# vsergeev/luaradio

Hardware: AMD Instinct MI355X
Metric: MSamples/s per block (128-tap complex FIR headline) + WBFM chain end-to-end (higher is better)
Workload: dtype f32

## Files before the change

### luaradio_amd/csrc/kernels_channelizer.h

```cpp
#pragma once
#include "common.h"
#include "kernels_fir.h"

#ifndef LRHIP_CHAN_EXP
#define LRHIP_CHAN_EXP 0
#endif

namespace lrhip {

#ifndef LRHIP_CHAN_INTERLEAVE
#define LRHIP_CHAN_INTERLEAVE 1
#endif
#ifndef LRHIP_CHAN_RT
#define LRHIP_CHAN_RT 1
#endif
#ifndef LRHIP_CHAN_KSLAB
#define LRHIP_CHAN_KSLAB 32
#endif
constexpr int CHAN_RT = LRHIP_CHAN_RT;
constexpr int CHAN_MT = 64 * CHAN_RT;
constexpr int CHAN_KSLAB = LRHIP_CHAN_KSLAB;

template <int NCT>
__global__ __launch_bounds__(256, CHAN_RT == 1 ? 2 : 1) void channelizer_kernel(const float *__restrict__ hist, const float *__restrict__ x,
                                                             const float *__restrict__ W, float *__restrict__ y,
                                                             int M, long n, long nframes, long first)
{
    constexpr int K2 = 16 * NCT;
    constexpr int K = K2 / 2;
    constexpr int DROW = K2 + 2;
    constexpr int WROW = K2 + 16;
    extern __shared__ __attribute__((aligned(16))) float lds[];
    const int tid = threadIdx.x, lane = tid & 63, wave = tid >> 6;
    const int col = lane & 15, kq = lane >> 4;
    const long f0 = (long)blockIdx.x * CHAN_MT;
    const int nsamp = (CHAN_MT - 1) * K + M;
    const int nflt = 2 * nsamp;
    float *ldsD = lds;
    const int dsize = ((nflt + 2 * (nflt / K2) + 2 + 3) / 4) * 4;
    float *ldsW = lds + dsize;

    const long p0 = first + f0 * K;
    const long xlo = p0 - (M - 1);
    if (xlo >= 0 && xlo + nsamp <= n && ((reinterpret_cast<uintptr_t>(x + 2 * xlo) & 15) == 0)) {
        const float4 *src = reinterpret_cast<const float4 *>(x + 2 * xlo);
        for (int i4 = tid; i4 < nflt / 4; i4 += 256) {
            float4 v = src[i4];
            int a = 4 * i4, p = a + 2 * (a / K2);
            *reinterpret_cast<float2 *>(ldsD + p) = make_float2(v.x, v.y);
            *reinterpret_cast<float2 *>(ldsD + p + 2) = make_float2(v.z, v.w);
        }
        for (int a = (nflt / 4) * 4 + tid; a < nflt; a += 256) ldsD[a + 2 * (a / K2)] = x[2 * xlo + a];
    } else {
        for (int r = tid; r < nsamp; r += 256) {
            int a = 2 * r, p = a + 2 * (a / K2);
            ldsD[p] = stream_at<2>(hist, x, p0 + r, 0, M, n);
            ldsD[p + 1] = stream_at<2>(hist, x, p0 + r, 1, M, n);
        }
    }

    constexpr int SLAB_F4 = CHAN_KSLAB * K2 / 4;
    constexpr int UW = (SLAB_F4 + 255) / 256;
    const float4 *W4 = reinterpret_cast<const float4 *>(W);
    static_assert(UW <= 8, "W slab prefetch: at most 8 float4 per thread");
    float4 w0, w1, w2, w3, w4, w5, w6, w7;
#define LR_CHAN_FOR8(OP) OP(0) OP(1) OP(2) OP(3) OP(4) OP(5) OP(6) OP(7)
#define LR_CHAN_LOAD(U)                                                                          \
    if (U < UW) {                                                                                \
        int i4 = tid + U * 256;                                                                  \
        w##U = W4[wbase + (i4 < SLAB_F4 ? i4 : SLAB_F4 - 1)];                                    \
    }
#define LR_CHAN_PUT(U)                                                                           \
    if (U < UW) {                                                                                \
        int i4 = tid + U * 256;                                                                  \
        if (i4 < SLAB_F4) *reinterpret_cast<float4 *>(wdst + ((4 * i4) / K2) * WROW + (4 * i4) % K2) = w##U; \
    }
    {
        const size_t wbase = 0;
        float *wdst = ldsW;
        LR_CHAN_FOR8(LR_CHAN_LOAD)
        LR_CHAN_FOR8(LR_CHAN_PUT)
    }
    __syncthreads();

    f32x4 acc[CHAN_RT][NCT];
#pragma unroll
    for (int r = 0; r < CHAN_RT; r++)
#pragma unroll
        for (int c = 0; c < NCT; c++) acc[r][c] = (f32x4){0.f, 0.f, 0.f, 0.f};
    const float *abase = ldsD + DROW * (wave * 16 * CHAN_RT + col) + kq;
    const int nslabs = 2 * M / CHAN_KSLAB;
    for (int s = 0; s < nslabs; s++) {
        const float *wcur = ldsW + (s & 1) * (CHAN_KSLAB * WROW);
#if LRHIP_CHAN_EXP == 1
        const bool more = false;
#else
        const bool more = s + 1 < nslabs;
#endif
        if (more) {
            const size_t wbase = (size_t)(s + 1) * SLAB_F4;
            LR_CHAN_FOR8(LR_CHAN_LOAD)
        }
        const float *ap = abase + CHAN_KSLAB * s + 2 * ((CHAN_KSLAB * s) / K2);
        const float *bp = wcur + kq * WROW + col;
        constexpr int NST = CHAN_KSLAB / 4;
        float av[2][CHAN_RT], bv[2][NCT];
        auto fetch = [&](int buf, int st) {
#pragma unroll
            for (int r = 0; r < CHAN_RT; r++) av[buf][r] = ap[16 * r * DROW + 4 * st];
#pragma unroll
            for (int c = 0; c < NCT; c++) bv[buf][c] = bp[4 * st * WROW + 16 * c];
        };
        fetch(0, 0);
#pragma unroll
        for (int st = 0; st < NST; st++) {
#if LRHIP_CHAN_INTERLEAVE
            if (st + 1 < NST) fetch((st + 1) & 1, st + 1);
#pragma unroll
            for (int c = 0; c < NCT; c++)
#pragma unroll
                for (int r = 0; r < CHAN_RT; r++)
                    acc[r][c] = __builtin_amdgcn_mfma_f32_16x16x4f32(av[st & 1][r], bv[st & 1][c], acc[r][c], 0, 0, 0);
#pragma unroll
            for (int i = 0; i < NCT * CHAN_RT; i++) {
                __builtin_amdgcn_sched_group_barrier(0x008, 1, 0);
                __builtin_amdgcn_sched_group_barrier(0x100, 1, 0);
            }
            __builtin_amdgcn_sched_barrier(0);
#else
            if (st + 1 < NST) fetch((st + 1) & 1, st + 1);
            __builtin_amdgcn_sched_barrier(0);
#pragma unroll
            for (int c = 0; c < NCT; c++)
#pragma unroll
                for (int r = 0; r < CHAN_RT; r++)
                    acc[r][c] = __builtin_amdgcn_mfma_f32_16x16x4f32(av[st & 1][r], bv[st & 1][c], acc[r][c], 0, 0, 0);
            __builtin_amdgcn_sched_barrier(0);
#endif
        }
        if (more) {
            float *wdst = ldsW + ((s + 1) & 1) * (CHAN_KSLAB * WROW);
            LR_CHAN_FOR8(LR_CHAN_PUT)
        }
#if LRHIP_CHAN_EXP != 1
        __syncthreads();
#endif
    }

#pragma unroll
    for (int rt = 0; rt < CHAN_RT; rt++)
#pragma unroll
        for (int c = 0; c < NCT; c++)
#pragma unroll
            for (int r = 0; r < 4; r++) {
                long f = f0 + (wave * CHAN_RT + rt) * 16 + 4 * kq + r;
                if (f < nframes) y[f * K2 + 16 * c + col] = acc[rt][c][r];
            }
}

#undef LR_CHAN_FOR8
#undef LR_CHAN_LOAD
#undef LR_CHAN_PUT

}
```

### luaradio_amd/csrc/stage_pfb.h

```cpp
#pragma once

struct PfbChannelizerStage : lrhip_stage {
    int seek(unsigned long long, unsigned long long *) override { return set_error("seek: not supported by the channelizer stage"); }
    long memory() const override { return -1; }
    int M = 0, K = 0, log2k = 0, P = 0, R = 1, D = 0;
    DeviceBuf taps, tw, hist[2];
    int cur = 0;
    unsigned long index = 0;
    unsigned phase = 0;
    const char *kind() const override { return "pfb_channelizer"; }
    unsigned long max_output(unsigned long n) const override { return (n / D + 1) * K; }
    static const char *refusal(unsigned ntaps, unsigned nchannels)
    {
        if (nchannels < 8 || nchannels > 4096 || (nchannels & (nchannels - 1))) return "pfb_channelizer: nchannels must be a power of two in [8, 4096]";
        const unsigned hi = 64 * nchannels < 65536 ? 64 * nchannels : 65536;
        if (ntaps < nchannels || ntaps > hi) return "pfb_channelizer: ntaps must be in [nchannels, min(64 * nchannels, 65536)]";
        return nullptr;
    }
    static const char *refusal(unsigned ntaps, unsigned nchannels, unsigned oversample)
    {
        if (oversample != 1 && oversample != 2 && oversample != 4) return "pfb_channelizer: oversample must be 1, 2 or 4";
        return refusal(ntaps, nchannels);
    }
    int frames_per_tile() const { return K <= 256 ? PFB_TILE_SMALL / K : K == 512 ? 8 : K == 1024 ? 4 : PFB_TILE_LARGE / K; }
    int frames_per_group() const { return K <= 1024 ? frames_per_tile() : PFB_SCRATCH / K; }
    int reset() override
    {
        cur = 0; index = 0; phase = 0;
        size_t hb = (size_t)(M - 1) * 2 * sizeof(float);
        return (zero_fill(hist[0], hb) || zero_fill(hist[1], hb)) ? -1 : 0;
    }
    template <int F, int NT>
    int launch(const float *x, long n, float *y, long nframes)
    {
        const int T = frames_per_tile(), G = frames_per_group();
        size_t lds_bytes = ((size_t)(T + G) * K + K / 2) * sizeof(float2);
        auto kern = pfb_channelizer_kernel<F, NT>;
        if (kernel_allow_lds(kern, lds_bytes)) return -1;
        unsigned grid = (unsigned)((nframes + T - 1) / T);
        hipLaunchKernelGGL(kern, dim3(grid), dim3(NT), lds_bytes, ctx().stream, (const float *)hist[cur].p, x, (const float *)taps.p,
                           (const float2 *)tw.p, y, M, log2k, P, T, G, n, nframes, (long)index);
        LR_LAUNCH_CHECK();
        return 0;
    }
    template <int RR, int F, int NT>
    int launch_oversampled(int T, int G, const float *x, long n, float *y, long nframes)
    {
        if (F > 1 && T % (RR * F)) return set_error("pfb_channelizer: a tile of %d frames does not hold blocks of %d frames in %d classes", T, F, RR);
        size_t lds_bytes = ((size_t)(T + G) * K + K / 2) * sizeof(float2);
        auto kern = pfb_oversampled_kernel<RR, F, NT>;
        if (kernel_allow_lds(kern, lds_bytes)) return -1;
        unsigned grid = (unsigned)((nframes + T - 1) / T);
        hipLaunchKernelGGL(kern, dim3(grid), dim3(NT), lds_bytes, ctx().stream, (const float *)hist[cur].p, x, (const float *)taps.p,
                           (const float2 *)tw.p, y, M, log2k, P, T, G, n, nframes, (long)index, (int)phase);
        LR_LAUNCH_CHECK();
        return 0;
    }
    int launch_oversampled_by_k(const float *x, long n, float *y, long nframes)
    {
        const int Ts = PFB_TILE_SMALL / K;
        if (R == 2) switch (log2k) {
            case 7: return launch_oversampled<2, 8, 256>(16, 16, x, n, y, nframes);
            case 8: return launch_oversampled<2, 4, 256>(8, 8, x, n, y, nframes);
            case 9: return launch_oversampled<2, 4, 1024>(8, 8, x, n, y, nframes);
            case 10: return launch_oversampled<2, 2, 512>(4, 4, x, n, y, nframes);
            case 11: return launch_oversampled<2, 4, 1024>(8, 1, x, n, y, nframes);
            case 12: return launch_oversampled<2, 1, 1024>(2, 1, x, n, y, nframes);
            default: return launch_oversampled<2, 8, 256>(Ts, Ts, x, n, y, nframes);
        }
        switch (log2k) {
            case 7: return launch_oversampled<4, 4, 256>(16, 16, x, n, y, nframes);
            case 8: return launch_oversampled<4, 2, 256>(8, 8, x, n, y, nframes);
            case 9: return launch_oversampled<4, 4, 1024>(16, 4, x, n, y, nframes);
            case 10: return launch_oversampled<4, 2, 512>(8, 1, x, n, y, nframes);
            case 11: return launch_oversampled<4, 2, 1024>(8, 1, x, n, y, nframes);
            case 12: return launch_oversampled<4, 1, 1024>(2, 1, x, n, y, nframes);
            default: return launch_oversampled<4, 8, 256>(Ts, Ts, x, n, y, nframes);
        }
    }
    long run(const void *in_dev, unsigned long n_in, void *out_dev, unsigned long cap) override
    {
        long n = (long)n_in;
        if (n <= 0) return 0;
        long nframes = n_in > index ? (long)((n_in - index + D - 1) / D) : 0;
        if ((unsigned long)(nframes * K) > cap) return set_error("pfb_channelizer: output capacity %lu < %ld", cap, nframes * K);
        const float *x = (const float *)in_dev;
        if (nframes > 0) {
            float *y = (float *)out_dev;
            int rc = R > 1 ? launch_oversampled_by_k(x, n, y, nframes)
                   : K <= 256 ? launch<8, 256>(x, n, y, nframes) : K == 512 ? launch<8, 1024>(x, n, y, nframes) : K == 1024 ? launch<4, 512>(x, n, y, nframes)
                   : K == 2048 ? launch<4, 1024>(x, n, y, nframes) : launch<2, 1024>(x, n, y, nframes);
            if (rc) return rc;
        }
        unsigned grid = grid_for((unsigned long)(M - 1) * 2, 256);
        hipLaunchKernelGGL(fir_history_kernel<2>, dim3(grid), dim3(256), 0, ctx().stream, (const float *)hist[cur].p, x, (float *)hist[cur ^ 1].p, M, n);
        LR_LAUNCH_CHECK();
        cur ^= 1;
        index = index + (unsigned long)nframes * D - n_in;
        phase = (unsigned)((phase + nframes) % R);
        return nframes * K;
    }
};

static ChannelizerStage *channelizer_build(const float *taps, unsigned ntaps, unsigned nchannels)
{
    auto q = new_stage<ChannelizerStage>();
    if (!q) return nullptr;
    int M = (int)ntaps, K = (int)nchannels, K2 = 2 * K;
    q->M = M; q->K = K;
    q->in_size = q->out_size = 8;
    std::vector<float> W((size_t)2 * M * K2);
    const double PI2 = 6.283185307179586476925286766559;
    for (int i = 0; i < M; i++)
        for (int c = 0; c < K; c++) {
            int j = M - 1 - i;
            double a = PI2 * (double)(((long)c * j) % K) / K, h = taps[j];
            float gr = (float)(h * std::cos(a)), gi = (float)(h * std::sin(a));
            W[(size_t)(2 * i) * K2 + 2 * c] = gr;
            W[(size_t)(2 * i + 1) * K2 + 2 * c] = -gi;
            W[(size_t)(2 * i) * K2 + 2 * c + 1] = gi;
            W[(size_t)(2 * i + 1) * K2 + 2 * c + 1] = gr;
        }
    if (upload(q->W, W.data(), W.size() * sizeof(float))) return nullptr;
    if (q->reset()) return nullptr;
    return q.release();
}
```

### luaradio_amd/csrc/stage_resample.h

```cpp
#pragma once

struct ResampleStage : lrhip_stage {
    int S = 2, M = 0, L = 1, HQ = 0;
    unsigned long D = 1;
    float c = 1.f;
    DeviceBuf d_taps, d_ttab, hist[2];
    int cur = 0;
    uint64_t Q0 = 0, m0 = 0;
    int interp_J = 0;
    static bool rational_supported(int L, unsigned long D) { return (L == 3 && D == 2) || (L == 2 && D == 3) || (L == 4 && D == 3) || (L == 3 && D == 4) || (L == 5 && D == 4) || (L == 4 && D == 5); }
    static int resample_rounds(long ntiles, long slots)
    {
        static const char *e = getenv("LRHIP_RESAMPLE_ROUNDS");
        if (e) return atoi(e) < 0 ? 0 : atoi(e);
        return persistent_rounds(ntiles, slots, 1);
    }
    static constexpr int SPAN_MAX = 6144;
    const char *kind() const override { return "resample"; }
    unsigned long max_output(unsigned long n) const override { return (n * (unsigned long)L) / D + 2; }
    int seek(unsigned long long n0, unsigned long long *n0_out) override
    {
        if (reset()) return -1;
        Q0 = n0;
        m0 = (n0 * (uint64_t)L + D - 1) / D;
        *n0_out = m0;
        return 0;
    }
    long memory() const override { return HQ; }
    void rate(unsigned long *num, unsigned long *den) const override { *num = D; *den = (unsigned long)L; }
    static bool fits(int M, int L, unsigned long D) { return L >= 1 && 256 * D / (unsigned long)L + (unsigned long)((M - 1) / L) + 4 <= (unsigned long)SPAN_MAX; }
    int reset() override
    {
        cur = 0; Q0 = 0; m0 = 0;
        size_t hb = (size_t)(HQ > 0 ? HQ : 1) * S * sizeof(float);
        return (zero_fill(hist[0], hb) || zero_fill(hist[1], hb)) ? -1 : 0;
    }
    long run(const void *in_dev, unsigned long n, void *out_dev, unsigned long cap) override
    {
        if (!n) return 0;
        uint64_t hi = (Q0 + n) * (uint64_t)L;
        uint64_t m_end = (hi + D - 1) / D;
        long n_out = (long)(m_end - m0);
        if ((unsigned long)n_out > cap) return set_error("resample: output capacity %lu < %ld", cap, n_out);
        const float *h = (const float *)hist[cur].p;
        float *ho = (float *)hist[cur ^ 1].p;
        if (interp_J > 0 && D == 1 && ((uintptr_t)in_dev & 7) == 0 && ((uintptr_t)out_dev & 7) == 0) {
            auto gi = [&](auto kern, size_t lds_bytes, int tq) -> int {
                const long ntiles = ((long)n + tq - 1) / tq, slots = chip_slots(kern, FIP_NT, lds_bytes);
                if (slots < 0) return -1;
                const int rounds = resample_rounds(ntiles, slots);
                hipLaunchKernelGGL(kern, dim3(persistent_grid(ntiles, slots, rounds)), dim3(FIP_NT), lds_bytes, ctx().stream, h, (const float *)in_dev, (const float *)d_ttab.p,
                                   (float *)out_dev, (long)n, HQ, c, ho, ablation_bits("LRHIP_INTERP_DBG"), rounds);
                return 0;
            };
#define LR_INTERP(LL, JJ) gi(fir_interp_kernel<LL, JJ>, (size_t)FipGeom<LL, JJ>::LDS_FLOATS * sizeof(float), FipGeom<LL, JJ>::TQ)
            int rc = L == 2 ? LR_INTERP(2, 64) : L == 3 ? LR_INTERP(3, 43) : L == 4 ? LR_INTERP(4, 32) : LR_INTERP(5, 26);
#undef LR_INTERP
            if (rc) return rc;
            LR_LAUNCH_CHECK();
            cur ^= 1;
            Q0 += n;
            m0 = m_end;
            return n_out;
        }
        static const bool no_rational = getenv("LRHIP_NO_RATIONAL_WIN") != nullptr;
        if (!no_rational && interp_J > 0 && D > 1 && ((uintptr_t)in_dev & 7) == 0 && ((uintptr_t)out_dev & 7) == 0) {
            auto gr = [&](auto kern, size_t lds_bytes, int tq) -> int {
                const long ntiles = ((long)n + (long)(Q0 % D) + tq - 1) / tq, slots = chip_slots(kern, 256, lds_bytes);
                if (slots < 0) return -1;
                const int rounds = resample_rounds(ntiles, slots);
                hipLaunchKernelGGL(kern, dim3(persistent_grid(ntiles, slots, rounds)), dim3(256), lds_bytes, ctx().stream, h, (const float *)in_dev, (const float *)d_ttab.p,
                                   (float *)out_dev, (long)n, n_out, m0, Q0, HQ, c, ho, rounds);
                return 0;
            };
#define LR_RAT(LL, DD, JJ, RR) gr(fir_rational_kernel<LL, DD, JJ, RR>, (size_t)FrrGeom<LL, DD, JJ, RR>::LDS_FLOATS * sizeof(float), FrrGeom<LL, DD, JJ, RR>::TQ)
            int rc = (L == 3 && D == 2) ? LR_RAT(3, 2, 43, 6) : (L == 2 && D == 3) ? LR_RAT(2, 3, 64, 9) : (L == 4 && D == 3) ? LR_RAT(4, 3, 32, 6)
                   : (L == 3 && D == 4) ? LR_RAT(3, 4, 43, 8) : (L == 5 && D == 4) ? LR_RAT(5, 4, 26, 8) : LR_RAT(4, 5, 32, 10);
#undef LR_RAT
            if (rc) return rc;
            LR_LAUNCH_CHECK();
            cur ^= 1;
            Q0 += n;
            m0 = m_end;
            return n_out;
        }
        int span_cap = (int)(256 * D / (unsigned long)L) + (M - 1) / L + 4;
        size_t lds_bytes = ((size_t)((((M - 1) / L + 1) * L + 3) & ~3) + (size_t)span_cap * S) * sizeof(float);
        auto go = [&](auto kern) -> int {
            if (kernel_allow_lds(kern, lds_bytes)) return -1;
            unsigned grid = n_out > 0 ? (unsigned)((n_out + 255) / 256) : 1;
            hipLaunchKernelGGL(kern, dim3(grid), dim3(256), lds_bytes, ctx().stream, h, (const float *)in_dev, (const float *)d_taps.p, (float *)out_dev, M, L,
                               (long)D, (long)n, n_out, m0, Q0, HQ, c, span_cap, ho);
            return 0;
        };
        int rc = S == 2 ? go(fir_resample_kernel<2>) : go(fir_resample_kernel<1>);
        if (rc) return rc;
        LR_LAUNCH_CHECK();
        cur ^= 1;
        Q0 += n;
        m0 = m_end;
        return n_out;
    }
};

struct ChannelizerStage : lrhip_stage {
    int seek(unsigned long long, unsigned long long *) override { return set_error("seek: not supported by the channelizer stage"); }
    long memory() const override { return -1; }
    int M = 0, K = 0;
    DeviceBuf W, hist[2];
    int cur = 0;
    unsigned long index = 0;
    const char *kind() const override { return "channelizer"; }
    unsigned long max_output(unsigned long n) const override { return (n / K + 1) * K; }
    int reset() override
    {
        cur = 0; index = 0;
        size_t hb = (size_t)(M - 1) * 2 * sizeof(float);
        return (zero_fill(hist[0], hb) || zero_fill(hist[1], hb)) ? -1 : 0;
    }
    template <int NCT>
    int launch(const float *x, long n, float *y, long nframes)
    {
        constexpr int K2 = 16 * NCT;
        int nflt = 2 * ((CHAN_MT - 1) * K + M);
        size_t dsize = (size_t)((nflt + 2 * (nflt / K2) + 2 + 3) / 4) * 4;
        size_t lds_bytes = (dsize + (size_t)2 * CHAN_KSLAB * (K2 + 16)) * sizeof(float);
        auto kern = channelizer_kernel<NCT>;
        if (kernel_allow_lds(kern, lds_bytes)) return -1;
        unsigned grid = (unsigned)((nframes + CHAN_MT - 1) / CHAN_MT);
        hipLaunchKernelGGL(kern, dim3(grid), dim3(256), lds_bytes, ctx().stream, (const float *)hist[cur].p, x, (const float *)W.p, y, M, n,
                           nframes, (long)index);
        LR_LAUNCH_CHECK();
        return 0;
    }
    long run(const void *in_dev, unsigned long n_in, void *out_dev, unsigned long cap) override
    {
        long n = (long)n_in;
        if (n <= 0) return 0;
        long nframes = n_in > index ? (long)((n_in - index + K - 1) / K) : 0;
        if ((unsigned long)(nframes * K) > cap) return set_error("channelizer: output capacity %lu < %ld", cap, nframes * K);
        const float *x = (const float *)in_dev;
        if (nframes > 0) {
            int rc = K == 32 ? launch<4>(x, n, (float *)out_dev, nframes) : launch<8>(x, n, (float *)out_dev, nframes);
            if (rc) return rc;
        }
        unsigned grid = grid_for((unsigned long)(M - 1) * 2, 256);
        hipLaunchKernelGGL(fir_history_kernel<2>, dim3(grid), dim3(256), 0, ctx().stream, (const float *)hist[cur].p, x, (float *)hist[cur ^ 1].p, M, n);
        LR_LAUNCH_CHECK();
        cur ^= 1;
        index = index + (unsigned long)nframes * K - n_in;
        return nframes * K;
    }
};
```

Baseline: 316,100.

## Factor channelizer into polyphase taps times real DFT matrix on MFMA

Replaces the dense per-tap complex weight matrix (2M x 2K) with a factorisation: the input samples are scaled by the prototype taps, then multiplied by a compact K x K real cos/sin matrix on MFMA, with conjugate-symmetry butterflies producing the complex channel outputs in the epilogue. This shrinks the weight operand from about 4MK floats to K*K floats plus M taps, removing the double-buffered global W slab streaming and per-slab barriers. Taps are staged in LDS and the DFT matrix is read from global/cache by default. Separate real and imaginary accumulators change the instruction mix and precision ordering, and the half-width tile count (NCT halved) changes the launch configuration.

```diff
diff --git a/luaradio_amd/csrc/kernels_channelizer.h b/luaradio_amd/csrc/kernels_channelizer.h
--- a/luaradio_amd/csrc/kernels_channelizer.h
+++ b/luaradio_amd/csrc/kernels_channelizer.h
@@ -2,34 +2,44 @@
 #include "common.h"
 #include "kernels_fir.h"
 
-#ifndef LRHIP_CHAN_EXP
-#define LRHIP_CHAN_EXP 0
-#endif
-
 namespace lrhip {
 
-#ifndef LRHIP_CHAN_INTERLEAVE
-#define LRHIP_CHAN_INTERLEAVE 1
-#endif
 #ifndef LRHIP_CHAN_RT
 #define LRHIP_CHAN_RT 1
 #endif
-#ifndef LRHIP_CHAN_KSLAB
-#define LRHIP_CHAN_KSLAB 32
+#ifndef LRHIP_CHAN_T_LDS
+#define LRHIP_CHAN_T_LDS 0
+#endif
+#ifndef LRHIP_CHAN_H_LDS
+#define LRHIP_CHAN_H_LDS 1
 #endif
 constexpr int CHAN_RT = LRHIP_CHAN_RT;
 constexpr int CHAN_MT = 64 * CHAN_RT;
-constexpr int CHAN_KSLAB = LRHIP_CHAN_KSLAB;
+constexpr int CHAN_DPAD = 4;
+constexpr int CHAN_TPAD = 16;
+
+__host__ __device__ inline int chan_data_floats(int K, int M)
+{
+    const int nsamp = (CHAN_MT - 1) * K + M;
+    return 2 * nsamp + CHAN_DPAD * ((nsamp + K - 1) / K);
+}
+__host__ __device__ inline int chan_lds_floats(int K, int M)
+{
+    return chan_data_floats(K, M) + (LRHIP_CHAN_H_LDS ? M : 0) + (LRHIP_CHAN_T_LDS ? K * (K + CHAN_TPAD) : 0);
+}
+
+typedef float chan_f32x2 __attribute__((ext_vector_type(2)));
 
 template <int NCT>
 __global__ __launch_bounds__(256, CHAN_RT == 1 ? 2 : 1) void channelizer_kernel(const float *__restrict__ hist, const float *__restrict__ x,
-                                                             const float *__restrict__ W, float *__restrict__ y,
+                                                             const float *__restrict__ T, const float *__restrict__ h, float *__restrict__ y,
                                                              int M, long n, long nframes, long first)
 {
-    constexpr int K2 = 16 * NCT;
-    constexpr int K = K2 / 2;
-    constexpr int DROW = K2 + 2;
-    constexpr int WROW = K2 + 16;
+    constexpr int K = 16 * NCT;
+    constexpr int K2 = 2 * K;
+    constexpr int NH = NCT / 2;
+    constexpr int PITCH = K2 + CHAN_DPAD;
+    constexpr int TROW = LRHIP_CHAN_T_LDS ? K + CHAN_TPAD : K;
     extern __shared__ __attribute__((aligned(16))) float lds[];
     const int tid = threadIdx.x, lane = tid & 63, wave = tid >> 6;
     const int col = lane & 15, kq = lane >> 4;
@@ -37,129 +47,102 @@
     const int nsamp = (CHAN_MT - 1) * K + M;
     const int nflt = 2 * nsamp;
     float *ldsD = lds;
-    const int dsize = ((nflt + 2 * (nflt / K2) + 2 + 3) / 4) * 4;
-    float *ldsW = lds + dsize;
+    float *ldsH = lds + chan_data_floats(K, M);
+    float *ldsT = ldsH + (LRHIP_CHAN_H_LDS ? M : 0);
+    auto pos = [](int u) { return 2 * u + CHAN_DPAD * (u / K); };
 
     const long p0 = first + f0 * K;
     const long xlo = p0 - (M - 1);
     if (xlo >= 0 && xlo + nsamp <= n && ((reinterpret_cast<uintptr_t>(x + 2 * xlo) & 15) == 0)) {
         const float4 *src = reinterpret_cast<const float4 *>(x + 2 * xlo);
-        for (int i4 = tid; i4 < nflt / 4; i4 += 256) {
-            float4 v = src[i4];
-            int a = 4 * i4, p = a + 2 * (a / K2);
-            *reinterpret_cast<float2 *>(ldsD + p) = make_float2(v.x, v.y);
-            *reinterpret_cast<float2 *>(ldsD + p + 2) = make_float2(v.z, v.w);
-        }
-        for (int a = (nflt / 4) * 4 + tid; a < nflt; a += 256) ldsD[a + 2 * (a / K2)] = x[2 * xlo + a];
+        for (int i4 = tid; i4 < nflt / 4; i4 += 256) *reinterpret_cast<float4 *>(ldsD + pos(2 * i4)) = src[i4];
     } else {
         for (int r = tid; r < nsamp; r += 256) {
-            int a = 2 * r, p = a + 2 * (a / K2);
+            const int p = pos(r);
             ldsD[p] = stream_at<2>(hist, x, p0 + r, 0, M, n);
             ldsD[p + 1] = stream_at<2>(hist, x, p0 + r, 1, M, n);
         }
     }
-
-    constexpr int SLAB_F4 = CHAN_KSLAB * K2 / 4;
-    constexpr int UW = (SLAB_F4 + 255) / 256;
-    const float4 *W4 = reinterpret_cast<const float4 *>(W);
-    static_assert(UW <= 8, "W slab prefetch: at most 8 float4 per thread");
-    float4 w0, w1, w2, w3, w4, w5, w6, w7;
-#define LR_CHAN_FOR8(OP) OP(0) OP(1) OP(2) OP(3) OP(4) OP(5) OP(6) OP(7)
-#define LR_CHAN_LOAD(U)                                                                          \
-    if (U < UW) {                                                                                \
-        int i4 = tid + U * 256;                                                                  \
-        w##U = W4[wbase + (i4 < SLAB_F4 ? i4 : SLAB_F4 - 1)];                                    \
-    }
-#define LR_CHAN_PUT(U)                                                                           \
-    if (U < UW) {                                                                                \
-        int i4 = tid + U * 256;                                                                  \
-        if (i4 < SLAB_F4) *reinterpret_cast<float4 *>(wdst + ((4 * i4) / K2) * WROW + (4 * i4) % K2) = w##U; \
-    }
-    {
-        const size_t wbase = 0;
-        float *wdst = ldsW;
-        LR_CHAN_FOR8(LR_CHAN_LOAD)
-        LR_CHAN_FOR8(LR_CHAN_PUT)
-    }
+    if (LRHIP_CHAN_H_LDS)
+        for (int i = tid; i < M; i += 256) ldsH[i] = h[i];
+    if (LRHIP_CHAN_T_LDS)
+        for (int i = tid; i < K * K; i += 256) ldsT[(i / K) * TROW + (i % K)] = T[i];
     __syncthreads();
 
-    f32x4 acc[CHAN_RT][NCT];
+    f32x4 accR[CHAN_RT][NCT], accI[CHAN_RT][NCT];
 #pragma unroll
-    for (int r = 0; r < CHAN_RT; r++)
+    for (int rt = 0; rt < CHAN_RT; rt++)
 #pragma unroll
-        for (int c = 0; c < NCT; c++) acc[r][c] = (f32x4){0.f, 0.f, 0.f, 0.f};
-    const float *abase = ldsD + DROW * (wave * 16 * CHAN_RT + col) + kq;
-    const int nslabs = 2 * M / CHAN_KSLAB;
-    for (int s = 0; s < nslabs; s++) {
-        const float *wcur = ldsW + (s & 1) * (CHAN_KSLAB * WROW);
-#if LRHIP_CHAN_EXP == 1
-        const bool more = false;
-#else
-        const bool more = s + 1 < nslabs;
-#endif
-        if (more) {
-            const size_t wbase = (size_t)(s + 1) * SLAB_F4;
-            LR_CHAN_FOR8(LR_CHAN_LOAD)
+        for (int t = 0; t < NCT; t++) accR[rt][t] = accI[rt][t] = (f32x4){0.f, 0.f, 0.f, 0.f};
+
+    const float *tsrc = (LRHIP_CHAN_T_LDS ? ldsT : T) + kq * TROW + col;
+    const float *hsrc = (LRHIP_CHAN_H_LDS ? ldsH : h) + kq;
+    const int ubase = (wave * 16 * CHAN_RT + col) * K + (M - 1) - kq;
+    float bv[NCT], bn[NCT];
+#pragma unroll
+    for (int t = 0; t < NCT; t++) bv[t] = bn[t] = tsrc[16 * t];
+    for (int r0 = 0; r0 < K; r0 += 4) {
+        const int np = (M - r0 + K - 1) / K;
+        if (np <= 0) break;
+        if (r0 + 4 < K) {
+#pragma unroll
+            for (int t = 0; t < NCT; t++) bn[t] = tsrc[(r0 + 4) * TROW + 16 * t];
         }
-        const float *ap = abase + CHAN_KSLAB * s + 2 * ((CHAN_KSLAB * s) / K2);
-        const float *bp = wcur + kq * WROW + col;
-        constexpr int NST = CHAN_KSLAB / 4;
-        float av[2][CHAN_RT], bv[2][NCT];
-        auto fetch = [&](int buf, int st) {
+        const float *ap = ldsD + pos(ubase - r0);
+        const float *hp = hsrc + r0;
+        chan_f32x2 a0[CHAN_RT], a1[CHAN_RT];
+        float h0, h1;
+        auto fetch = [&](chan_f32x2 (&a)[CHAN_RT], float &hv, int p) {
 #pragma unroll
-            for (int r = 0; r < CHAN_RT; r++) av[buf][r] = ap[16 * r * DROW + 4 * st];
+            for (int rt = 0; rt < CHAN_RT; rt++) a[rt] = *reinterpret_cast<const chan_f32x2 *>(ap + 16 * rt * PITCH - p * PITCH);
+            hv = hp[p * K];
+        };
+        auto mac = [&](const chan_f32x2 (&a)[CHAN_RT], float hv) {
 #pragma unroll
-            for (int c = 0; c < NCT; c++) bv[buf][c] = bp[4 * st * WROW + 16 * c];
+            for (int rt = 0; rt < CHAN_RT; rt++) {
+                const chan_f32x2 s = a[rt] * (chan_f32x2){hv, hv};
+#pragma unroll
+                for (int t = 0; t < NCT; t++) {
+                    accR[rt][t] = __builtin_amdgcn_mfma_f32_16x16x4f32(s.x, bv[t], accR[rt][t], 0, 0, 0);
+                    accI[rt][t] = __builtin_amdgcn_mfma_f32_16x16x4f32(s.y, bv[t], accI[rt][t], 0, 0, 0);
+                }
+            }
         };
-        fetch(0, 0);
+        fetch(a0, h0, 0);
+        for (int p = 0; p < np; p += 2) {
+            fetch(a1, h1, p + 1 < np ? p + 1 : p);
+            __builtin_amdgcn_sched_barrier(0);
+            mac(a0, h0);
+            __builtin_amdgcn_sched_barrier(0);
+            if (p + 1 >= np) break;
+            fetch(a0, h0, p + 2 < np ? p + 2 : p + 1);
+            __builtin_amdgcn_sched_barrier(0);
+            mac(a1, h1);
+            __builtin_amdgcn_sched_barrier(0);
+        }
 #pragma unroll
-        for (int st = 0; st < NST; st++) {
-#if LRHIP_CHAN_INTERLEAVE
-            if (st + 1 < NST) fetch((st + 1) & 1, st + 1);
-#pragma unroll
-            for (int c = 0; c < NCT; c++)
-#pragma unroll
-                for (int r = 0; r < CHAN_RT; r++)
-                    acc[r][c] = __builtin_amdgcn_mfma_f32_16x16x4f32(av[st & 1][r], bv[st & 1][c], acc[r][c], 0, 0, 0);
-#pragma unroll
-            for (int i = 0; i < NCT * CHAN_RT; i++) {
-                __builtin_amdgcn_sched_group_barrier(0x008, 1, 0);
-                __builtin_amdgcn_sched_group_barrier(0x100, 1, 0);
-            }
-            __builtin_amdgcn_sched_barrier(0);
-#else
-            if (st + 1 < NST) fetch((st + 1) & 1, st + 1);
-            __builtin_amdgcn_sched_barrier(0);
-#pragma unroll
-            for (int c = 0; c < NCT; c++)
-#pragma unroll
-                for (int r = 0; r < CHAN_RT; r++)
-                    acc[r][c] = __builtin_amdgcn_mfma_f32_16x16x4f32(av[st & 1][r], bv[st & 1][c], acc[r][c], 0, 0, 0);
-            __builtin_amdgcn_sched_barrier(0);
-#endif
-        }
-        if (more) {
-            float *wdst = ldsW + ((s + 1) & 1) * (CHAN_KSLAB * WROW);
-            LR_CHAN_FOR8(LR_CHAN_PUT)
-        }
-#if LRHIP_CHAN_EXP != 1
-        __syncthreads();
-#endif
+        for (int t = 0; t < NCT; t++) bv[t] = bn[t];
     }
 
 #pragma unroll
     for (int rt = 0; rt < CHAN_RT; rt++)
 #pragma unroll
-        for (int c = 0; c < NCT; c++)
+        for (int tp = 0; tp < NH; tp++)
 #pragma unroll
             for (int r = 0; r < 4; r++) {
-                long f = f0 + (wave * CHAN_RT + rt) * 16 + 4 * kq + r;
-                if (f < nframes) y[f * K2 + 16 * c + col] = acc[rt][c][r];
+                const long f = f0 + (wave * CHAN_RT + rt) * 16 + 4 * kq + r;
+                if (f >= nframes) continue;
+                const int c = 16 * tp + col;
+                const float pr = accR[rt][tp][r], pi = accI[rt][tp][r], qr = accR[rt][NH + tp][r], qi = accI[rt][NH + tp][r];
+                float2 *yf = reinterpret_cast<float2 *>(y + f * K2);
+                if (c == 0) {
+                    yf[0] = make_float2(pr + 0.f * pi, pi + 0.f * pr);
+                    yf[K / 2] = make_float2(qr + 0.f * qi, qi + 0.f * qr);
+                } else {
+                    yf[c] = make_float2(pr - qi, pi + qr);
+                    yf[K - c] = make_float2(pr + qi, pi - qr);
+                }
             }
 }
 
-#undef LR_CHAN_FOR8
-#undef LR_CHAN_LOAD
-#undef LR_CHAN_PUT
-
 }
diff --git a/luaradio_amd/csrc/stage_pfb.h b/luaradio_amd/csrc/stage_pfb.h
--- a/luaradio_amd/csrc/stage_pfb.h
+++ b/luaradio_amd/csrc/stage_pfb.h
@@ -106,22 +106,19 @@
 {
     auto q = new_stage<ChannelizerStage>();
     if (!q) return nullptr;
-    int M = (int)ntaps, K = (int)nchannels, K2 = 2 * K;
+    int M = (int)ntaps, K = (int)nchannels;
     q->M = M; q->K = K;
     q->in_size = q->out_size = 8;
-    std::vector<float> W((size_t)2 * M * K2);
+    std::vector<float> T((size_t)K * K);
     const double PI2 = 6.283185307179586476925286766559;
-    for (int i = 0; i < M; i++)
-        for (int c = 0; c < K; c++) {
-            int j = M - 1 - i;
-            double a = PI2 * (double)(((long)c * j) % K) / K, h = taps[j];
-            float gr = (float)(h * std::cos(a)), gi = (float)(h * std::sin(a));
-            W[(size_t)(2 * i) * K2 + 2 * c] = gr;
-            W[(size_t)(2 * i + 1) * K2 + 2 * c] = -gi;
-            W[(size_t)(2 * i) * K2 + 2 * c + 1] = gi;
-            W[(size_t)(2 * i + 1) * K2 + 2 * c + 1] = gr;
+    for (int r = 0; r < K; r++)
+        for (int col = 0; col < K; col++) {
+            int c = col < K / 2 ? col : col == K / 2 ? K / 2 : col - K / 2;
+            double a = PI2 * (double)((c * r) % K) / K;
+            T[(size_t)r * K + col] = (float)(col <= K / 2 ? std::cos(a) : std::sin(a));
         }
-    if (upload(q->W, W.data(), W.size() * sizeof(float))) return nullptr;
+    if (upload(q->T, T.data(), T.size() * sizeof(float))) return nullptr;
+    if (upload(q->taps, taps, (size_t)M * sizeof(float))) return nullptr;
     if (q->reset()) return nullptr;
     return q.release();
 }
diff --git a/luaradio_amd/csrc/stage_resample.h b/luaradio_amd/csrc/stage_resample.h
--- a/luaradio_amd/csrc/stage_resample.h
+++ b/luaradio_amd/csrc/stage_resample.h
@@ -107,7 +107,7 @@
     int seek(unsigned long long, unsigned long long *) override { return set_error("seek: not supported by the channelizer stage"); }
     long memory() const override { return -1; }
     int M = 0, K = 0;
-    DeviceBuf W, hist[2];
+    DeviceBuf T, taps, hist[2];
     int cur = 0;
     unsigned long index = 0;
     const char *kind() const override { return "channelizer"; }
@@ -121,15 +121,12 @@
     template <int NCT>
     int launch(const float *x, long n, float *y, long nframes)
     {
-        constexpr int K2 = 16 * NCT;
-        int nflt = 2 * ((CHAN_MT - 1) * K + M);
-        size_t dsize = (size_t)((nflt + 2 * (nflt / K2) + 2 + 3) / 4) * 4;
-        size_t lds_bytes = (dsize + (size_t)2 * CHAN_KSLAB * (K2 + 16)) * sizeof(float);
+        size_t lds_bytes = (size_t)chan_lds_floats(16 * NCT, M) * sizeof(float);
         auto kern = channelizer_kernel<NCT>;
         if (kernel_allow_lds(kern, lds_bytes)) return -1;
         unsigned grid = (unsigned)((nframes + CHAN_MT - 1) / CHAN_MT);
-        hipLaunchKernelGGL(kern, dim3(grid), dim3(256), lds_bytes, ctx().stream, (const float *)hist[cur].p, x, (const float *)W.p, y, M, n,
-                           nframes, (long)index);
+        hipLaunchKernelGGL(kern, dim3(grid), dim3(256), lds_bytes, ctx().stream, (const float *)hist[cur].p, x, (const float *)T.p, (const float *)taps.p, y, M,
+                           n, nframes, (long)index);
         LR_LAUNCH_CHECK();
         return 0;
     }
@@ -141,7 +138,7 @@
         if ((unsigned long)(nframes * K) > cap) return set_error("channelizer: output capacity %lu < %ld", cap, nframes * K);
         const float *x = (const float *)in_dev;
         if (nframes > 0) {
-            int rc = K == 32 ? launch<4>(x, n, (float *)out_dev, nframes) : launch<8>(x, n, (float *)out_dev, nframes);
+            int rc = K == 32 ? launch<2>(x, n, (float *)out_dev, nframes) : launch<4>(x, n, (float *)out_dev, nframes);
             if (rc) return rc;
         }
         unsigned grid = grid_for((unsigned long)(M - 1) * 2, 256);
```

After: 315,900. No clear change (-0.1%).
